# carlostojal/NDT-Net

Hardware: AMD Instinct MI355X
Metric: clouds/sec NDT preprocess+PointNet fwd, 100k pts->1000 NDs, batch=16 (higher is better)
Workload: dtype f64 NDT; PointNet fp32-accurate split-bf16x3 (6 products) on 11 per-point layers, fp32 MFMA on the K=16 first layers and the TNet / seg-bias FC layers

## Files before the change

include/ndnet_pointnet.h:

```cpp
#ifndef NDNET_POINTNET_H_
#define NDNET_POINTNET_H_
#include <stdint.h>

#ifdef __cplusplus
extern "C" {
#endif

#define NDNET_PN_MAX_LAYERS 5

typedef struct ndnet_pn_layer {
  const float* w;
  int64_t w_cloud_stride;
  const float* bias;
  int64_t bias_cloud_stride;
  int32_t K, N;
  int32_t relu;
  int32_t prec;
  int32_t fuse_next;
} ndnet_pn_layer;

typedef struct ndnet_pn_chain {
  const float* x;
  int32_t x_ld;
  int32_t in_cols;
  int32_t num_points;
  int32_t num_layers;
  ndnet_pn_layer L[NDNET_PN_MAX_LAYERS];
  int32_t mode;
  int32_t out_cols;
  float* gmax;
  int32_t gmax_ld;
  int32_t max_width;
  int32_t max_width2;
  float* out;
  float* clear;
  int64_t clear_count;
  const float* head_h2;
  int32_t head_ld, head_K;
  const float* head_w3;
  const float* head_b3;
  const float* head_basis;
  int32_t head_kin, head_nout;
  float* head_t1;
  const float* fold_t2;
  int32_t fold_ld;
  float* fold_out_w;
  float* fold_out_b;
} ndnet_pn_chain;

int ndnet_pn_chain_run(const ndnet_pn_chain *args, int batch, void *stream);
int ndnet_pn_chain_run_t32(const ndnet_pn_chain *args, int batch, void *stream);

int ndnet_pn_debug_stamps(unsigned long long *host, int wgs);
int ndnet_pn_debug_stamps_clear(void);

int ndnet_pn_fc_run(const float *in, int ld_in, const float *W, const float *bias, float *out, int ld_out,
                    int batch, int K, int N, int relu, void *stream);
int ndnet_pn_fc_mfma_run(const float *in, int ld_in, const float *Wf, const float *bias, float *out, int ld_out,
                         int batch, int K, int N, int relu, void *stream);
int ndnet_pn_cls_head_run(const float *in, int ld_in, const float *Wf, const float *bias, float *probs,
                          int ld_probs, float *logits, int ld_logits, int batch, int K, int N, int out_cols,
                          float *clear, int64_t clear_count, void *stream);
#define NDNET_FOLD_WT 0
#define NDNET_FOLD_FRAG 1
#define NDNET_FOLD_FRAG6 2
#define NDNET_FOLD_ROWS 3
#define NDNET_FOLD_BASIS 4
#define NDNET_FOLD_BIAS 5
typedef struct ndnet_pn_fold_job {
  const float *w;
  const float *bias;
  const float *gamma, *beta, *mean, *var;
  void *out;
  int32_t kind;
  int32_t N, K;
  int32_t ld, k0;
  int32_t Kp, Np;
  int32_t eye;
  float eps;
  int32_t reserved;
  int64_t block0;
} ndnet_pn_fold_job;
int ndnet_pn_fold_prepare(ndnet_pn_fold_job *host_jobs, int num_jobs, int64_t *num_blocks);
int ndnet_pn_fold_run(const ndnet_pn_fold_job *device_jobs, int num_jobs, int64_t num_blocks, void *stream);

int ndnet_pn_head3_run(const float *h2, int ld_h, const float *W3, const float *b3, const float *basis,
                       float *t1, float *w1f, int batch, int K, int kin, int nout, void *stream);

int ndnet_pn_fold_t2_run(const float *w1f, int w1_stride, const float *b1, const float *t2, int t2_ld, float *outf,
                         float *outb, int batch, void *stream);

#ifdef __cplusplus
}
#endif

#endif
```

ndt-net_amd/csrc/pointnet_kernels.hip:

```cpp
#include <hip/hip_runtime.h>
#include <math.h>
#include <stdint.h>
#include <stdio.h>
#include <stdlib.h>

#include "../../include/ndnet_pointnet.h"

namespace {

#ifndef NDNET_PN_TILE
#define NDNET_PN_TILE 64
#endif
constexpr int kP = NDNET_PN_TILE;
#ifndef NDNET_PN_WAVES
#define NDNET_PN_WAVES (NDNET_PN_TILE / 4)
#endif
constexpr int kWaves = NDNET_PN_WAVES;
constexpr int kThreads = 64 * kWaves;
constexpr int kRowBlocks = kP / 16;
static_assert(kP == 64 || kP == 32, "64- or 32-point tiles");
constexpr int kFuseNC = 64;
constexpr int kPadF = 8;
constexpr int kPadB = 16;
#ifndef NDNET_PN_PLANE_SWZ
// ... 1155 lines not shown
  return ((int64_t)((n >> 4) * KG + (k >> 4)) * 64 + ((k >> 2) & 3) * 16 + (n & 15)) * 4 + (k & 3);
}

template <int WPO>
__global__ void __launch_bounds__(256) k_pn_fc_split(const float* __restrict__ in, int ld_in,
                                                     const float* __restrict__ W, const float* __restrict__ bias,
                                                     float* __restrict__ out, int ld_out, int B, int N, int relu) {
  constexpr int K = 256 * WPO, OPW = 4 / WPO;
  __shared__ float s_part[4][16];
  const int lane = threadIdx.x & 63, wave = threadIdx.x >> 6;
  const int o = wave / WPO, wq = wave % WPO;
  const int n = blockIdx.x * OPW + o;
  const int nn = n < N ? n : N - 1;
  const int c4 = wq * 64 + lane;
  const f32x4 wv = reinterpret_cast<const f32x4*>(W + (int64_t)nn * K)[c4];
  f32x4 xv[16];
#pragma unroll
  for (int b = 0; b < 16; b++) xv[b] = reinterpret_cast<const f32x4*>(in + (int64_t)(b < B ? b : 0) * ld_in)[c4];
  float acc[16];
#pragma unroll
  for (int b = 0; b < 16; b++) {
    const f32x4 pr = xv[b] * wv;
    acc[b] = (pr[0] + pr[1]) + (pr[2] + pr[3]);
  }
#pragma unroll
  for (int b = 0; b < 16; b++)
    for (int off = 32; off > 0; off >>= 1) acc[b] += __shfl_xor(acc[b], off, 64);
  if (WPO > 1) {
    if (lane < 16) {
      float v = 0.0f;
#pragma unroll
      for (int b = 0; b < 16; b++) v = lane == b ? acc[b] : v;
      s_part[wave][lane] = v;
    }
    __syncthreads();
    if (wq != 0) return;
    if (lane < 16) {
      float v = 0.0f;
#pragma unroll
      for (int q = 0; q < WPO; q++) v += s_part[wave + q][lane];
      acc[0] = v;
    }
  } else if (lane < 16) {
    float v = 0.0f;
#pragma unroll
    for (int b = 0; b < 16; b++) v = lane == b ? acc[b] : v;
    acc[0] = v;
  }
  if (lane < B && n < N) {
    float v = acc[0] + bias[n];
    if (relu) v = fmaxf(v, 0.0f);
    out[(int64_t)lane * ld_out + n] = v;
  }
}

__global__ void __launch_bounds__(1024) k_pn_fold_t2(const float* __restrict__ w1f, int w1_stride,
                                                     const float* __restrict__ b1, const float* __restrict__ t2,
                                                     int t2_ld, float* __restrict__ outf, float* __restrict__ outb) {
  const int b = blockIdx.x, e = threadIdx.x;
  __shared__ float s_w[13 * 64];
  __shared__ float s_t[64 * 64];
  {
    const float* wb = w1f + (int64_t)b * w1_stride;
    if (e < 16 * 64) {
      const int cb = e >> 8, ln = (e >> 2) & 63, k = 4 * (ln >> 4) + (e & 3), n = 16 * cb + (ln & 15);
      const float v = wb[e];
      if (k < 12) s_w[k * 64 + n] = v;
    }
    if (e < 64) s_w[12 * 64 + e] = b1[e];
    const f32x4* tb = reinterpret_cast<const f32x4*>(t2 + (int64_t)b * t2_ld);
    reinterpret_cast<f32x4*>(s_t)[e] = tb[e];
  }
  __syncthreads();
  if (e < 13 * 64) {
    const int r = e >> 6, n = e & 63;
    float acc = 0.0f;
#pragma unroll 16
    for (int i = 0; i < 64; i++) acc = fmaf(s_w[r * 64 + i], s_t[i * 64 + n], acc);
    if (r < 12) outf[(int64_t)b * 1024 + ((((n >> 4) * 64 + ((r >> 2) & 3) * 16 + (n & 15)) << 2) + (r & 3))] = acc;
    else outb[(int64_t)b * 64 + n] = acc;
  }
}

__global__ void __launch_bounds__(256) k_pn_head3(const float* __restrict__ h2, int ld_h, const float* __restrict__ W3,
                                                  const float* __restrict__ b3, const float* __restrict__ basis,
                                                  float* __restrict__ t1_out, float* __restrict__ w1f, int K, int kin,
                                                  int nout) {
  __shared__ float s_t[9];
  const int b = blockIdx.x;
  const int lane = threadIdx.x & 63, wave = threadIdx.x >> 6;
  const float* h = h2 + (int64_t)b * ld_h;
  for (int o = wave; o < 9; o += 4) {
    float acc = 0.0f;
    for (int k = lane; k < K; k += 64) acc += h[k] * W3[(int64_t)o * K + k];
    for (int off = 32; off > 0; off >>= 1) acc += __shfl_xor(acc, off, 64);
    if (lane == 0) {
      s_t[o] = acc + b3[o];
      t1_out[b * 9 + o] = acc + b3[o];
    }
  }
  const int M = kin * nout, total = 16 * nout;
  auto kn = [&](int e, int& k, int& n) {
    const int cb = e >> 8, ln = (e >> 2) & 63;
    k = 4 * (ln >> 4) + (e & 3);
    n = 16 * cb + (ln & 15);
  };
  constexpr int kE = 4;
  float bas[kE][9];
#pragma unroll
  for (int i = 0; i < kE; i++) {
    const int e = threadIdx.x + i * blockDim.x;
    int k, n;
    kn(e, k, n);
#pragma unroll
    for (int a = 0; a < 9; a++) bas[i][a] = (e < total && k < kin) ? basis[a * M + k * nout + n] : 0.0f;
  }
  __syncthreads();
#pragma unroll
  for (int i = 0; i < kE; i++) {
    const int e = threadIdx.x + i * blockDim.x;
    if (e < total) {
      float acc = 0.0f;
#pragma unroll
      for (int a = 0; a < 9; a++) acc += s_t[a] * bas[i][a];
      w1f[(int64_t)b * total + e] = acc;
    }
  }
  for (int e = threadIdx.x + kE * blockDim.x; e < total; e += blockDim.x) {
    int k, n;
    kn(e, k, n);
    float acc = 0.0f;
    if (k < kin) {
#pragma unroll
      for (int a = 0; a < 9; a++) acc += s_t[a] * basis[a * M + k * nout + n];
    }
    w1f[(int64_t)b * total + e] = acc;
  }
}

#if NDNET_PN_TILE == 64
constexpr int kFoldThreads = 256;

__device__ inline uint16_t fold_bf16(float x) {
  uint32_t u = __float_as_uint(x);
  if ((u & 0x7fffffffu) > 0x7f800000u) return (uint16_t)((u >> 16) | 0x40u);
  return (uint16_t)((u + 0x7fffu + ((u >> 16) & 1u)) >> 16);
}

__device__ inline float fold_w(const ndnet_pn_fold_job& J, int n, int k) {
#pragma clang fp contract(off)
  if (n >= J.N || k >= J.K) return 0.0f;
  const float w = J.w[(int64_t)n * J.ld + J.k0 + k];
  if (!J.gamma) return w;
  return w * (J.gamma[n] / sqrtf(J.var[n] + J.eps));
}

__host__ __device__ inline int64_t fold_units(const ndnet_pn_fold_job& J) {
  switch (J.kind) {
    case NDNET_FOLD_WT: return (int64_t)J.Kp * J.Np;
    case NDNET_FOLD_FRAG: return (int64_t)J.Kp * J.Np / 4;
    case NDNET_FOLD_FRAG6: return (int64_t)J.Kp * J.Np / 8;
    case NDNET_FOLD_ROWS: return (int64_t)J.N * J.K;
    case NDNET_FOLD_BASIS: return (int64_t)9 * J.K * J.N;
    default: return J.Np;
  }
}
// ... 75 lines not shown
    }
  }
}
#endif

#if NDNET_PN_TILE == 64
int fc_mfma_cbw(int nb, int ngmax) {
  static const int cap = [] {
    const char* e = getenv("NDNET_PN_FC_CBW");
    return e ? atoi(e) : 4;
  }();
  for (int c = cap >= 4 ? 4 : cap >= 2 ? 2 : 1; c > 1; c >>= 1)
    if (nb % c == 0 && nb / c >= 32 && ngmax * c <= kFcMaxG) return c;
  return 1;
}
#endif

}

extern "C" {

#if NDNET_PN_TILE == 64
int ndnet_pn_fc_mfma_run(const float* in, int ld_in, const float* Wf, const float* bias, float* out, int ld_out,
                         int batch, int K, int N, int relu, void* stream) {
  if (!in || !Wf || !bias || !out || batch <= 0 || batch > 16 || K <= 0 || K % 16 || K > 16 * kFcWaves * kFcMaxG ||
      N <= 0 || N % 16 || ld_in % 4 || ld_in < K || ld_out < N || ((uintptr_t)in | (uintptr_t)Wf) % 16)
    return -20;
  const int KG = K / 16, nb = N / 16, ngmax = (KG + kFcWaves - 1) / kFcWaves;
  const int cbw = fc_mfma_cbw(nb, ngmax);
  const f32x4* wf = reinterpret_cast<const f32x4*>(Wf);
  hipStream_t st = (hipStream_t)stream;
  if (cbw == 4)
    k_pn_fc_mfma<4><<<nb / 4, kFcWaves * 64, 0, st>>>(in, ld_in, wf, bias, out, ld_out, batch, KG, relu);
  else if (cbw == 2)
    k_pn_fc_mfma<2><<<nb / 2, kFcWaves * 64, 0, st>>>(in, ld_in, wf, bias, out, ld_out, batch, KG, relu);
  else
    k_pn_fc_mfma<1><<<nb, kFcWaves * 64, 0, st>>>(in, ld_in, wf, bias, out, ld_out, batch, KG, relu);
  return hipGetLastError() == hipSuccess ? 0 : -21;
}

int ndnet_pn_cls_head_run(const float* in, int ld_in, const float* Wf, const float* bias, float* probs, int ld_probs,
                          float* logits, int ld_logits, int batch, int K, int N, int out_cols, float* clear,
                          int64_t clear_count, void* stream) {
  if (!in || !Wf || !bias || !probs || batch <= 0 || K <= 0 || K % 16 || K > 16 * kClsMaxG || N <= 0 || N % 16 ||
      N > 1024 || out_cols < 1 || out_cols > N || ld_in % 4 || ld_in < K || ld_probs < out_cols ||
      (logits && ld_logits < out_cols) || ((uintptr_t)in | (uintptr_t)Wf) % 16 || clear_count < 0 ||
      (!clear && clear_count))
    return -20;
  k_pn_cls_head<<<(batch + 15) / 16, kClsWaves * 64, (size_t)16 * N * sizeof(float), (hipStream_t)stream>>>(
      in, ld_in, reinterpret_cast<const f32x4*>(Wf), bias, probs, ld_probs, logits, ld_logits, batch, K / 16, N,
      out_cols, clear, clear_count);
  return hipGetLastError() == hipSuccess ? 0 : -21;
}

int ndnet_pn_fc_run(const float* in, int ld_in, const float* W, const float* bias, float* out, int ld_out, int batch,
                    int K, int N, int relu, void* stream) {
  if (!in || !W || !bias || !out || batch <= 0 || batch > 16 || K <= 0 || K % 4 || N <= 0 || ld_in % 4 ||
      ld_in < K || ld_out < N || ((uintptr_t)in | (uintptr_t)W) % 16)
    return -20;
  hipStream_t st = (hipStream_t)stream;
  switch (K % 256 == 0 && K <= 1024 ? K / 256 : 0) {
    case 2: k_pn_fc_split<2><<<(N + 1) / 2, 256, 0, st>>>(in, ld_in, W, bias, out, ld_out, batch, N, relu); break;
    case 4: k_pn_fc_split<4><<<N, 256, 0, st>>>(in, ld_in, W, bias, out, ld_out, batch, N, relu); break;
    default: k_pn_fc<<<(N + 3) / 4, 256, 0, st>>>(in, ld_in, W, bias, out, ld_out, batch, K, N, relu);
  }
  return hipGetLastError() == hipSuccess ? 0 : -21;
}

int ndnet_pn_head3_run(const float* h2, int ld_h, const float* W3, const float* b3, const float* basis, float* t1,
                       float* w1f, int batch, int K, int kin, int nout, void* stream) {
  if (!h2 || !W3 || !b3 || !basis || !t1 || !w1f || batch <= 0 || K <= 0 || ld_h < K || kin <= 0 || kin > 16 ||
      nout <= 0 || nout % 16)
    return -20;
  k_pn_head3<<<batch, 256, 0, (hipStream_t)stream>>>(h2, ld_h, W3, b3, basis, t1, w1f, K, kin, nout);
  return hipGetLastError() == hipSuccess ? 0 : -21;
}

int ndnet_pn_fold_t2_run(const float* w1f, int w1_stride, const float* b1, const float* t2, int t2_ld, float* outf,
                         float* outb, int batch, void* stream) {
  if (!w1f || !b1 || !t2 || !outf || !outb || batch <= 0 || w1_stride < 1024 || t2_ld < 4096 || t2_ld % 4 ||
      (uintptr_t)t2 % 16)
    return -20;
  k_pn_fold_t2<<<batch, 1024, 0, (hipStream_t)stream>>>(w1f, w1_stride, b1, t2, t2_ld, outf, outb);
  return hipGetLastError() == hipSuccess ? 0 : -21;
}

int ndnet_pn_fold_prepare(ndnet_pn_fold_job* jobs, int num_jobs, int64_t* num_blocks) {
  if (!jobs || num_jobs <= 0 || !num_blocks) return -20;
  int64_t blocks = 0;
  for (int i = 0; i < num_jobs; i++) {
    ndnet_pn_fold_job& J = jobs[i];
    const bool bn = J.gamma != nullptr;
    if (!J.out || (uintptr_t)J.out % 16 || J.kind < NDNET_FOLD_WT || J.kind > NDNET_FOLD_BIAS || J.N <= 0 ||
        (bn && (!J.beta || !J.mean || !J.var || !(J.eps >= 0.0f))) || (!bn && (J.beta || J.mean || J.var)))
      return -20;
    if (J.kind == NDNET_FOLD_BIAS) {
      if (!J.bias || J.Np < J.N || J.eye < 0 || (J.eye > 0 && J.eye * J.eye != J.N)) return -20;
    } else {
      if (!J.w || J.K <= 0 || J.k0 < 0 || J.ld < J.k0 + J.K) return -20;
      if (J.kind == NDNET_FOLD_WT && (J.Kp < J.K || J.Np < J.N)) return -20;
      if (J.kind == NDNET_FOLD_FRAG && (J.Kp < J.K || J.Np < J.N || J.Kp % 16 || J.Np % 16)) return -20;
      if (J.kind == NDNET_FOLD_FRAG6 && (J.Kp < J.K || J.Np < J.N || J.Kp % 32 || J.Np % 16)) return -20;
      if (J.kind == NDNET_FOLD_BASIS && J.K != 12) return -20;
    }
    J.block0 = blocks;
    blocks += (fold_units(J) + kFoldThreads - 1) / kFoldThreads;
  }
  if (blocks <= 0 || blocks > 0x7fffffff) return -20;
  *num_blocks = blocks;
  return 0;
}

int ndnet_pn_fold_run(const ndnet_pn_fold_job* jobs, int num_jobs, int64_t num_blocks, void* stream) {
  if (!jobs || num_jobs <= 0 || num_blocks <= 0 || num_blocks > 0x7fffffff) return -20;
  k_pn_fold<<<(unsigned)num_blocks, kFoldThreads, 0, (hipStream_t)stream>>>(jobs, num_jobs);
  return hipGetLastError() == hipSuccess ? 0 : -21;
}


int ndnet_pn_debug_stamps_clear(void) {
#ifdef NDNET_PN_STAMPS
  static unsigned long long zeros[kStampWgs][16];
  return hipMemcpyToSymbol(HIP_SYMBOL(g_pn_stamps), zeros, sizeof(zeros)) == hipSuccess ? 0 : -21;
#else
  return -20;
#endif
}

int ndnet_pn_debug_stamps(unsigned long long* host, int wgs) {
#ifdef NDNET_PN_STAMPS
  if (!host || wgs <= 0 || wgs > kStampWgs) return -20;
  if (hipDeviceSynchronize() != hipSuccess) return -21;
  return hipMemcpyFromSymbol(host, HIP_SYMBOL(g_pn_stamps), (size_t)wgs * 16 * sizeof(unsigned long long)) ==
                 hipSuccess ? 0 : -21;
#else
  (void)host; (void)wgs;
  return -20;
#endif
}
#endif

#define PN_ARG_FAIL()                                                                          \
  do {                                                                                         \
    fprintf(stderr, "ndnet_amd: chain launch: invalid argument (pointnet_kernels.hip:%d)\n", __LINE__); \
    return -20;                                                                                \
  } while (0)

#if NDNET_PN_TILE == 64
int ndnet_pn_chain_run(const ndnet_pn_chain* args, int batch, void* stream) {
#else
int ndnet_pn_chain_run_t32(const ndnet_pn_chain* args, int batch, void* stream) {
#endif
  if (!args || batch <= 0 || args->num_layers < 1 || args->num_layers > NDNET_PN_MAX_LAYERS || args->num_points <= 0 ||
      args->in_cols < 1 || args->in_cols > args->L[0].K || args->in_cols > args->x_ld)
    PN_ARG_FAIL();
  int w[2] = {args->L[0].K, 0};
  int pw1 = 0;
  bool has_fuse = false;
  int planes = 0, qprec = 0;
  int smode = 0;
  for (int l = 0; l < args->num_layers; l++) {
    const ndnet_pn_layer& L = args->L[l];
    if (!L.w || !L.bias || L.K <= 0 || L.K % 16 || L.N <= 0 || L.N % 32 || (L.N > 32 && L.N % 64) ||
        ((uintptr_t)L.w % 16) ||
        L.w_cloud_stride % 4)
      PN_ARG_FAIL();
// ... 88 lines not shown
```

ndt-net_amd/ndnet/_lib.py:

```python
from __future__ import annotations

import ctypes
import os

import torch

PKG = os.path.dirname(os.path.abspath(__file__))
ROOT = os.path.dirname(PKG)
LIB_PATH = os.environ.get("NDNET_AMD_LIB") or os.path.join(ROOT, "lib", "libndnet_amd.so")

NDNET_OK = 0
NDNET_ERR_ARG = -20
NDNET_ERR_HIP = -21
NDNET_ERR_SYNC = -22
POINT_FILL = {"none": 0, "nearest": 1}
SEG_CONF_LDS_MAX_COLS = 63
FPS_THREADS = 512
FPS_LDS_POINTS = {"float32": 12288, "float64": 6144}
FPS_REG_POINTS = {"float32": 100352, "float64": 49152}


class NdtStats(ctypes.Structure):
    _fields_ = [
        ("rc", ctypes.c_int32),
# ... 54 lines not shown
    "free_nds": (None, [_P, _UL]),
    "free_kl_divergences": (None, [_P]),
    "print_matrix": (None, [_P, _I, _I]),
    "ndnet_ndt_plan_create": (_I, [_I, _U64, _U64, _I, _U64, ctypes.POINTER(_P)]),
    "ndnet_ndt_plan_destroy": (None, [_P]),
    "ndnet_ndt_set_path": (_I, [_P, _I]),
    "ndnet_ndt_get_path": (_I, [_P]),
    "ndnet_ndt_get_front_lanes": (_I, [_P, ctypes.POINTER(_I), ctypes.POINTER(_I)]),
    "ndnet_ndt_take_sync_failures": (_I, [_P]),
    "ndnet_ndt_set_cu_share": (_I, [_P, _I, _I]),
    "ndnet_ndt_set_exact_counts": (_I, [_P, _I]),
    "ndnet_ndt_set_front_staged": (_I, [_P, _I]),
    "ndnet_ndt_get_front_staged": (_I, [_P]),
    "ndnet_ndt_set_run_part": (_I, [_P, _I]),
    "ndnet_ndt_set_lazy_list": (_I, [_P, _I]),
    "ndnet_ndt_set_heavy_threshold": (_I, [_P, ctypes.c_uint32]),
    "ndnet_ndt_set_welford_form": (_I, [_P, _I]),
    "ndnet_ndt_get_welford_form": (_I, [_P]),
    "ndnet_ndt_debug_set_sync_timeout": (_I, [_P, ctypes.c_uint64]),
    "ndnet_ndt_run": (_I, [_P, _P, _P, _P, _P, _P, _P]),
    "ndnet_ndt_run_f64": (_I, [_P, _P, _P, _P, _P, _P, _P, _P, _P]),
    "ndnet_ndt_prune": (_I, [_P, _P, _U64, _P, _P, _P, _P, _P, _P]),
    "ndnet_ndt_point_rows": (_I, [_P, _P, _P, _P, _U64, _I, _P]),
    "ndnet_ndt_run_counts": (_I, [_P, _P, _P, _P, _P, _P, _P, _P]),
    "ndnet_ndt_run_f64_counts": (_I, [_P, _P, _P, _P, _P, _P, _P, _P, _P, _P]),
    "ndnet_ndt_point_rows_counts": (_I, [_P, _P, _P, _P, _U64, _I, _P, _P]),
    "ndnet_seg_point_labels": (_I, [_P, _P, _I, _U64, _U64, _I, ctypes.c_int32, _P, _P, _P]),
    "ndnet_seg_point_labels_u8": (_I, [_P, _P, _I, _U64, _U64, _I, ctypes.c_uint8, _P, _P, _P]),
    "ndnet_seg_confusion": (_I, [_P, _P, _U64, _I, _P, _P]),
    "ndnet_seg_row_hist": (_I, [_P, _P, _I, _U64, _U64, _I, ctypes.c_int32, _P, _P]),
    "ndnet_fps_run": (_I, [_P, _I, _U64, _U64, _P, _P, _P, _P, _P]),
    "ndnet_fps_run_f64": (_I, [_P, _I, _U64, _U64, _P, _P, _P, _P, _P]),
    "ndnet_nearest_sample_run": (_I, [_P, _I, _U64, _P, _P, _U64, _P, _P, _P, _P]),
    "ndnet_pn_transform3_run": (_I, [_P, ctypes.c_int64, _P, _P, ctypes.c_int64, _I, _U64, _P]),
    "ndnet_aug_work_bytes": (ctypes.c_size_t, [_I, _U64]),
    "ndnet_aug_run": (_I, [_P, _P, _P, _P, _I, _U64, _P, _P, _P, _P, _P, _P, _P]),
    "ndnet_pts_unpack_i16": (_I, [_P, _P, _I, _U64, _P, _P, _P]),
    "ndnet_ndt_debug_dump": (_I, [_P, _I, _P, _P, _P, _P, _P, _P, _P, _P, _P, _P, _P, _P]),
    "ndnet_ndt_debug_set_epoch": (_I, [_P, ctypes.c_uint32]),
    "ndnet_ndt_debug_set_kl_fuse": (_I, [_P, _I]),
    "ndnet_ndt_debug_set_list_sort": (_I, [_P, _I]),
    "ndnet_ndt_debug_get_list_sort": (_I, [_P]),
    "ndnet_ndt_debug_kl_marks": (_I, [_P, _P]),
    "ndnet_ndt_debug_front_marks": (_I, [_P, _P]),
    "ndnet_ndt_debug_wq_marks": (_I, [_P, _P, ctypes.POINTER(ctypes.c_uint32)]),
    "ndnet_debug_lu_chain": (_I, [_P, ctypes.c_uint32, _I, _P, _P, _P, _P]),
    "ndnet_ndt_debug_front_wg_marks": (_I, [_P, _P, ctypes.POINTER(_I)]),
    "ndnet_ndt_set_timing": (_I, [_P, _I]),
    "ndnet_ndt_stage_ms": (_I, [_P, _P]),
    "ndnet_amd_version": (ctypes.c_char_p, []),
}


def lib() -> ctypes.CDLL:
    global _lib
    if _lib is None:
        if not os.path.exists(LIB_PATH):
            raise RuntimeError(f"{LIB_PATH} is missing: build it with `make -C {ROOT}` "
                               "(there is no CPU fallback)")
        _lib = ctypes.CDLL(LIB_PATH)
        for name, (res, args) in EXPORTS.items():
            fn = getattr(_lib, name)
            fn.restype = res
            fn.argtypes = args
        for name, (res, args) in {**POINTNET_EXPORTS, **TRAIN_EXPORTS}.items():
            fn = getattr(_lib, name)
            fn.restype = res
            fn.argtypes = args
    return _lib


POINTNET_EXPORTS: dict = {
    "ndnet_pn_chain_run": (_I, [_P, _I, _P]),
    "ndnet_pn_chain_run_t32": (_I, [_P, _I, _P]),
    "ndnet_pn_debug_stamps": (_I, [_P, _I]),
    "ndnet_pn_debug_stamps_clear": (_I, []),
    "ndnet_ply_count": (_I, [ctypes.c_char_p, _I, ctypes.POINTER(_U64)]),
    "ndnet_ply_read": (_I, [ctypes.c_char_p, _I, _I, _P, _P, _U64, ctypes.POINTER(_U64), _I]),
    "ndnet_pn_fc_run": (_I, [_P, _I, _P, _P, _P, _I, _I, _I, _I, _I, _P]),
    "ndnet_pn_fc_mfma_run": (_I, [_P, _I, _P, _P, _P, _I, _I, _I, _I, _I, _P]),
    "ndnet_pn_cls_head_run": (_I, [_P, _I, _P, _P, _P, _I, _P, _I, _I, _I, _I, _I, _P, ctypes.c_int64, _P]),
    "ndnet_pn_head3_run": (_I, [_P, _I, _P, _P, _P, _P, _P, _I, _I, _I, _I, _P]),
    "ndnet_pn_fold_t2_run": (_I, [_P, _I, _P, _P, _I, _P, _P, _I, _P]),
    "ndnet_pn_fold_prepare": (_I, [_P, _I, ctypes.POINTER(ctypes.c_int64)]),
    "ndnet_pn_fold_run": (_I, [_P, _I, ctypes.c_int64, _P]),
}


_I64 = ctypes.c_int64

TRAIN_EXPORTS: dict = {
    "ndnet_tr_gemm": (_I, [_P, _P, _P, _P, _I64, _I, _I, _I, _I64, _I64, _I64, _I64, _I64, _I64, _I, _I, _I, _I, _I,
                           _I, _P]),
    "ndnet_tr_sum_parts": (_I, [_P, _P, _I64, _I, _P]),
    "ndnet_tr_sum_parts_2d": (_I, [_P, _P, _I64, _I64, _I64, _I, _P]),
    "ndnet_tr_bn_fwd": (_I, [_P, _P, _P, _P, _P, _P, _P, _P, _I, _I, _I, ctypes.c_float, ctypes.c_float, _I, _P, _P,
                             _P, _P]),
    "ndnet_tr_bn_bwd": (_I, [_P, _P, _P, _P, _P, _P, _P, _P, _P, _P, _I, _I, _I, _I, _P, _P]),
    "ndnet_tr_chan_sum": (_I, [_P, _P, _I, _I, _I, _P]),
    "ndnet_tr_row_sum": (_I, [_P, _P, _I64, _I, _P]),
    "ndnet_tr_argmax_match": (_I, [_P, _P, _I64, _I, _P, _P]),
    "ndnet_tr_argmax_match_cm": (_I, [_P, _P, _I, _I, _I, _P, _P, _P]),
    "ndnet_row_argmax": (_I, [_P, _I64, _I, _P, _P]),
    "ndnet_tr_fc_fwd": (_I, [_P, _P, _P, _P, _P, _P, _P, _P, _P, _P, _P, _I, _I, _I, _I64, ctypes.c_float,
                             ctypes.c_float, _I, _I, _P, _P]),
    "ndnet_tr_fc_bwd_w": (_I, [_P, _P, _P, _P, _P, _P, _P, _P, _P, _P, _P, _P, _I, _I, _I, _I64, _I, _P]),
    "ndnet_tr_fc_bwd_x": (_I, [_P, _P, _P, _P, _I, _I, _I, _I64, _I, _P]),
    "ndnet_tr_point_transform": (_I, [_P, _P, _I, _P, _I, _P, _I, _I, _P]),
    "ndnet_tr_point_transform_bwd": (_I, [_P, _P, _I, _P, _I, _P, _I, _I, _P]),
    "ndnet_tr_log_softmax_c": (_I, [_P, _P, _I, _I, _I, _P]),
    "ndnet_tr_log_softmax_c_bwd": (_I, [_P, _P, _P, _I, _I, _I, _P]),
    "ndnet_tr_nll_onehot": (_I, [_P, _P, _P, _P, _I, _I, _I, _P]),
    "ndnet_tr_nll_onehot_bwd": (_I, [_P, _P, _P, _I, _I, _I, _P]),
    "ndnet_tr_nll_hist": (_I, [_P, _P, _P, _P, _P, _I, _I, _I, _P]),
    "ndnet_tr_nll_hist_bwd": (_I, [_P, _P, _P, _P, _I, _I, _I, _P]),
    "ndnet_tr_hist_match_cm": (_I, [_P, _P, _I, _I, _I, _P, _P, _P]),
    "ndnet_tr_adam": (_I, [_I, _P, _P, _P, _P, _P, _P, _P, ctypes.c_double, ctypes.c_double, ctypes.c_double,
                           ctypes.c_double, _P]),
}


def require_gpu() -> None:
    if not torch.cuda.is_available():
        raise RuntimeError("ndnet_amd needs a ROCm GPU (gfx950); none is visible and there is no CPU fallback")


def check(rc: int, what: str) -> None:
    if rc != NDNET_OK:
        raise RuntimeError(f"{what} failed with code {rc}")


def stream_ptr(device: torch.device | None = None) -> int:
    return torch.cuda.current_stream(device).cuda_stream
```

ndt-net_amd/ndnet/models/pointnet_hip.py:

```python
from __future__ import annotations

import ctypes
import os

import torch

from .. import _lib

MAX_LAYERS = 5
CHAIN_NAMES = ("A: TNet(3) 3-64-128-1024 + max", "B: conv1(t1) + TNet(64) 64-64-128-1024 + max",
               "C: conv1, conv2(t2), conv3 + max", "D: seg head 64-512-256-128-(C+1) + log_softmax")

chain_timing = None

MODES = {"x6": 1, "fp32": 1, "x3": 2, "bf16": 3}
PRECISION = SPLIT_BF16 = X6_PREC = None


def set_precision(mode: str) -> None:
    global PRECISION, SPLIT_BF16, X6_PREC
    if mode not in MODES:
        raise ValueError(f"unknown PointNet precision mode {mode!r}")
    PRECISION = mode
    SPLIT_BF16 = mode != "fp32"
# ... 298 lines not shown
                and all(t.is_contiguous() and t.dtype == torch.float32 for t in tensors if t.is_floating_point()))

    def refold(self) -> None:
        dev = self.c1wT.device
        if self._dev_jobs is None:
            arr = (_FoldJob * len(self.jobs))()
            for J, (kind, out, layer, bn, k0, K, Kp, Np, eye) in zip(arr, self.jobs):
                J.kind, J.out, J.N, J.K, J.ld, J.k0 = kind, out.data_ptr(), layer.weight.shape[0], K, \
                    layer.weight.shape[1], k0
                J.Kp, J.Np, J.eye = Kp, Np, eye
                if kind == 5:
                    J.bias = layer.bias.data_ptr()
                else:
                    J.w = layer.weight.data_ptr()
                if bn is not None:
                    J.gamma, J.beta = bn.weight.data_ptr(), bn.bias.data_ptr()
                    J.mean, J.var, J.eps = bn.running_mean.data_ptr(), bn.running_var.data_ptr(), bn.eps
            blocks = ctypes.c_int64()
            _lib.check(_lib.lib().ndnet_pn_fold_prepare(arr, len(arr), ctypes.byref(blocks)), "ndnet_pn_fold_prepare")
            self._dev_jobs = torch.frombuffer(bytearray(bytes(arr)), dtype=torch.uint8).to(dev)
            self._blocks = blocks.value
        rc = _lib.lib().ndnet_pn_fold_run(self._dev_jobs.data_ptr(), len(self.jobs), self._blocks,
                                          _lib.stream_ptr(dev))
        _lib.check(rc, "ndnet_pn_fold_run")


def _tensors(m) -> list:
    return list(m.parameters()) + list(m.buffers())


def _signature(tensors) -> tuple:
    return tuple((t.data_ptr(), t._version) for t in tensors)


def _fc_head(g: torch.Tensor, t: dict, dim: int, h1: torch.Tensor, h2: torch.Tensor, out: torch.Tensor):
    torch.addmm(t["c1"], g, t["f1"].t(), out=h1).relu_()
    torch.addmm(t["c2"], h1, t["f2"].t(), out=h2).relu_()
    torch.addmm(t["c3"], h2, t["f3"].t(), out=out)
    return out.view(-1, dim, dim)


def _build_chain(n: int, in_cols: int, layers, relus, mode: int, gmax=None, out_cols=0, fuse=(),
                 x_ld: int = 12) -> "_Chain":
    ch = _Chain()
    ch.x_ld = x_ld
    ch.in_cols = in_cols
    ch.num_points = n
    ch.num_layers = len(layers)
    widths = [layers[0][3], 8]
    for i, (w, stride, b, K, N, *prec) in enumerate(layers):
        L = ch.L[i]
        L.prec = prec[0] if prec else 0
        L.w = w.data_ptr()
        L.w_cloud_stride = stride
        L.K, L.N = K, N
        L.bias = b.data_ptr()
        L.bias_cloud_stride = b.stride(0) if b.dim() == 2 else 0
        L.relu = relus[i]
        L.fuse_next = 1 if i in fuse else 0
        if i in fuse:
            continue
        if i + 1 < len(layers) or mode == 1:
            widths[(i + 1) & 1] = max(widths[(i + 1) & 1], N)
    ch.mode = mode
    ch.out_cols = out_cols
    ch.gmax = gmax.data_ptr() if gmax is not None else None
    ch.gmax_ld = gmax.stride(0) if gmax is not None else 0
    ch.max_width, ch.max_width2 = widths
    return ch


TILE32 = os.environ.get("NDNET_PN_TILE32", "1") == "1"
_cus = {}


def _use_t32(B: int, n: int, device) -> bool:
    if not TILE32:
        return False
    if device not in _cus:
        _cus[device] = torch.cuda.get_device_properties(device).multi_processor_count
    return 2 * B * ((n + 63) // 64) <= _cus[device]


def _run_chain(ch: "_Chain", x: torch.Tensor, out=None) -> None:
    assert x.stride(1) == ch.x_ld and x.stride(2) == 1 and x.dtype == torch.float32
    ch.x = x.data_ptr()
    ch.out = out.data_ptr() if out is not None else None
    if _use_t32(x.shape[0], x.shape[1], x.device):
        rc = _lib.lib().ndnet_pn_chain_run_t32(ctypes.byref(ch), x.shape[0], _lib.stream_ptr(x.device))
        _lib.check(rc, "ndnet_pn_chain_run_t32")
        return
    rc = _lib.lib().ndnet_pn_chain_run(ctypes.byref(ch), x.shape[0], _lib.stream_ptr(x.device))
    _lib.check(rc, "ndnet_pn_chain_run")


def _chain_torch(x: torch.Tensor, n: int, in_cols: int, layers, relus, mode: int, gmax=None, out=None,
                 out_cols=0, fuse=()) -> None:
    h = x[..., :in_cols].float()
    k0 = layers[0][0].shape[-2]
    h = torch.nn.functional.pad(h, (0, k0 - in_cols))
    for i, (w, b) in enumerate(layers):
        h = torch.matmul(h, w[..., : h.shape[-1], :]) + (b[:, None, :] if b.dim() == 2 else b)
        if relus[i]:
            h = torch.relu(h)
    if mode == 0:
        gmax.copy_(torch.maximum(gmax, h.amax(dim=1)))
    else:
        out.copy_(torch.log_softmax(h[..., :out_cols], dim=2))


class _Workspace:

    def __init__(self, W: _Folded, B: int, N: int, dev, mode: str = None) -> None:
        self.W = W
        self.mode = PRECISION if mode is None else mode
        f32 = dict(dtype=torch.float32, device=dev)
        Fp = W.C_tail[0].shape[1]
        self.gbuf = torch.full((B, 2048 + Fp), float("-inf"), **f32)
        self.g1, self.g2, self.g3 = self.gbuf[:, :1024], self.gbuf[:, 1024:2048], self.gbuf[:, 2048:]
        self.h1, self.h2 = torch.empty((B, 512), **f32), torch.empty((B, 256), **f32)
        self.t1, self.t2 = torch.empty((B, 9), **f32), torch.empty((B, 4096), **f32)
        self.cvec = torch.empty((B, 512), **f32)
        kin = 3 if W.baseline else 12
        self.w1T = None if W.baseline else torch.empty((B, 12, 64), **f32)
        self.w1t2 = torch.empty((B, kin, 64), **f32)
        self.b1t2 = torch.empty((B, 64), **f32)
        self.w1f = None if W.baseline else torch.empty((B, 16 * 64), **f32)
        self.w1t2f = torch.zeros((B, 16 * 64), **f32)
        if W.baseline:
            self.xt = torch.zeros((B, N, 4), **f32)
            self.pts = None
        first = (W.c1T16, W.c1b) if W.baseline else (self.w1T, W.c1b)
        self.specs = [
            (3, W.A, (1, 1, 1), 0, dict(gmax=self.g1)),
            (kin, [first] + W.B_tail, (0, 1, 1, 1), 0, dict(gmax=self.g2)),
            (kin, [(self.w1t2, self.b1t2), W.C_mid, W.C_tail], (0, 0, 0), 0, dict(gmax=self.g3)),
        ]
        if W.seg:
            self.specs.append((kin, [(self.w1t2, self.b1t2), (W.s1aT, self.cvec)] + W.D_tail, (0, 1, 1, 1, 0), 1,
                               dict(out_cols=W.C1, fuse=(1,))))
        self.N = N
        self.structs = {}

    def hip_layers(self, mode: str) -> list:
        W = self.W

        def shared(wb):
            w, b = wb
            if mode != "fp32" and id(w) in W.frag6:
                return (W.frag6[id(w)], 0, b, w.shape[0], w.shape[1], MODES[mode])
            return (W.frag[id(w)], 0, b, w.shape[0], w.shape[1])

        L1 = shared((W.c1T16, W.c1b)) if W.baseline else (self.w1f, self.w1f.stride(0), W.c1b, 16, 64)
        LC = (self.w1t2f, self.w1t2f.stride(0), self.b1t2, 16, 64) if FOLD_T2_KERNEL and not W.baseline else L1
        layers = [
            [shared(x) for x in W.A],
            [L1] + [shared(x) for x in W.B_tail],
            [LC, shared(W.C_mid), shared(W.C_tail)],
        ]
        if W.seg:
            layers.append([(self.w1t2f, self.w1t2f.stride(0), self.b1t2, 16, 64), shared((W.s1aT, self.cvec))] +
                          [shared(x) for x in W.D_tail])
        return layers

    def chain(self, i: int, x: torch.Tensor, chain_fn=None, out=None) -> None:
        in_cols, layers, relus, mode, kw = self.specs[i]
        if chain_fn is not None:
            kw = dict(kw)
            if out is not None:
                kw["out"] = out
            chain_fn(x, self.N, in_cols, layers, relus, mode, **kw)
            return
        structs = self.structs.get(self.mode)
        W = self.W
        if structs is None:
            x_lds = (3, 4, 4, 4) if W.baseline else (12, 12, 12, 12)
            structs = self.structs[self.mode] = [_build_chain(self.N, s[0], hl, s[2], s[3], x_ld=xl, **s[4])
                                                 for s, hl, xl in zip(self.specs, self.hip_layers(self.mode), x_lds)]
            if W.seg:
                structs[3].clear = self.gbuf.data_ptr()
                structs[3].clear_count = self.gbuf.numel()
            if HEAD3_IN_CHAIN and not W.baseline:
                cb = structs[1]
                cb.head_h2, cb.head_ld, cb.head_K = self.h2.data_ptr(), self.h2.stride(0), self.h2.shape[1]
                cb.head_w3, cb.head_b3 = W.t1["f3"].data_ptr(), W.t1["c3"].data_ptr()
                cb.head_basis, cb.head_kin, cb.head_nout = W.t1_basis.data_ptr(), 12, 64
                cb.head_t1 = self.t1.data_ptr()
            if not FOLD_T2_KERNEL or W.baseline:
                cc = structs[2]
                cc.fold_t2, cc.fold_ld = self.t2.data_ptr(), self.t2.stride(0)
                cc.fold_out_w, cc.fold_out_b = self.w1t2f.data_ptr(), self.b1t2.data_ptr()
        if chain_timing is not None:
            e0, e1 = torch.cuda.Event(enable_timing=True), torch.cuda.Event(enable_timing=True)
            e0.record()
            _run_chain(structs[i], x, out)
            e1.record()
            chain_timing.append((i, e0, e1))
        else:
            _run_chain(structs[i], x, out)


def _folded(model):
    cache = model._hip
    if cache is None:
        tensors = _tensors(model)
        cache = model._hip = {"tensors": tensors, "sig": None, "stale": False}
    sig = _signature(cache["tensors"])
    cur = _tensors(model)
    replaced = len(cur) != len(cache["tensors"]) or any(a is not b for a, b in zip(cur, cache["tensors"]))
    if replaced or cache["sig"] != sig or cache["stale"]:
        W = cache.get("W")
        if W is not None and W.can_refold(_tensors(model)):
            W.refold()
        else:
            cache.update(tensors=_tensors(model), W=_Folded(model), ws={})
            sig = _signature(cache["tensors"])
        cache.update(sig=sig, stale=False)
    return cache


FOLD_T2_KERNEL = os.environ.get("NDNET_PN_FOLD_T2", "kernel") == "kernel"
HEAD3_IN_CHAIN = os.environ.get("NDNET_PN_HEAD3", "chain") == "chain"

FC_MFMA = os.environ.get("NDNET_PN_FC", "mfma") == "mfma"


def _fc(x: torch.Tensor, w: torch.Tensor, b: torch.Tensor, out: torch.Tensor, relu: bool, wf=None) -> None:
    B = x.shape[0]
    st = _lib.stream_ptr(x.device)
    for c0 in range(0, B, 16):
        n = min(16, B - c0)
        if FC_MFMA and wf is not None:
            rc = _lib.lib().ndnet_pn_fc_mfma_run(x[c0].data_ptr(), x.stride(0), wf.data_ptr(), b.data_ptr(),
                                                 out[c0].data_ptr(), out.stride(0), n, _pad(w.shape[1], 16),
                                                 w.shape[0], 1 if relu else 0, st)
            _lib.check(rc, "ndnet_pn_fc_mfma_run")
        else:
            rc = _lib.lib().ndnet_pn_fc_run(x[c0].data_ptr(), x.stride(0), w.data_ptr(), b.data_ptr(),
                                            out[c0].data_ptr(), out.stride(0), n, w.shape[1], w.shape[0],
                                            1 if relu else 0, st)
            _lib.check(rc, "ndnet_pn_fc_run")


def _glue_hip(W, ws, B: int):
    st = lambda: _lib.stream_ptr(ws.gbuf.device)

    def fc(x, w, b, out, relu):
        _fc(x, w, b, out, relu, W.fcf.get(id(w)))

    def head_a():
        t = W.t1
        fc(ws.g1, t["f1"], t["c1"], ws.h1, True)
        fc(ws.h1, t["f2"], t["c2"], ws.h2, True)
        if HEAD3_IN_CHAIN:
            return
        for c0 in range(0, B, 16):
            n = min(16, B - c0)
            rc = _lib.lib().ndnet_pn_head3_run(ws.h2[c0].data_ptr(), ws.h2.stride(0), t["f3"].data_ptr(),
                                               t["c3"].data_ptr(), W.t1_basis.data_ptr(), ws.t1[c0].data_ptr(),
                                               ws.w1f[c0].data_ptr(), n, 256, 12, 64, st())
            _lib.check(rc, "ndnet_pn_head3_run")

    def head_a_points():
        t = W.t1
        fc(ws.g1, t["f1"], t["c1"], ws.h1, True)
        fc(ws.h1, t["f2"], t["c2"], ws.h2, True)
        _fc(ws.h2, t["f3"], t["c3"], ws.t1, False, None)
        rc = _lib.lib().ndnet_pn_transform3_run(ws.pts.data_ptr(), ws.pts.stride(1), ws.t1.data_ptr(),
                                                ws.xt.data_ptr(), ws.xt.stride(1), B, ws.pts.shape[1], st())
        _lib.check(rc, "ndnet_pn_transform3_run")

    def head_b():
        t = W.t2
        fc(ws.g2, t["f1"], t["c1"], ws.h1, True)
        fc(ws.h1, t["f2"], t["c2"], ws.h2, True)
        fc(ws.h2, t["f3"], t["c3"], ws.t2, False)
        if FOLD_T2_KERNEL and not W.baseline:
            rc = _lib.lib().ndnet_pn_fold_t2_run(ws.w1f.data_ptr(), ws.w1f.stride(0), W.c1b.data_ptr(),
                                                 ws.t2.data_ptr(), ws.t2.stride(0), ws.w1t2f.data_ptr(),
                                                 ws.b1t2.data_ptr(), B, st())
            _lib.check(rc, "ndnet_pn_fold_t2_run")

    def seg_bias():
        fc(ws.g3[:, : W.F], W.s1g, W.s1b, ws.cvec, False)

    def cls_head(out):
        fc(ws.g3[:, : W.F], W.h1w, W.h1b, ws.h1, True)
        fc(ws.h1, W.h2w, W.h2b, ws.h2, True)
        rc = _lib.lib().ndnet_pn_cls_head_run(ws.h2.data_ptr(), ws.h2.stride(0), W.h3f.data_ptr(), W.h3b.data_ptr(),
                                              out.data_ptr(), out.stride(0), None, 0, B, ws.h2.shape[1], W.Cp, W.C,
                                              ws.gbuf.data_ptr(), ws.gbuf.numel(), st())
        _lib.check(rc, "ndnet_pn_cls_head_run")

    return (head_a_points if W.baseline else head_a), head_b, (seg_bias if W.seg else cls_head)


def _glue_torch(W, ws, B: int):
    def head_a():
        t1 = _fc_head(ws.g1, W.t1, 3, ws.h1, ws.h2, ws.t1)
        torch.matmul(t1.reshape(B, 9), W.t1_basis, out=ws.w1T.view(B, 12 * 64))

    def head_a_points():
        t1 = _fc_head(ws.g1, W.t1, 3, ws.h1, ws.h2, ws.t1)
        ws.xt[..., :3] = torch.nan_to_num(torch.bmm(ws.pts, t1.transpose(1, 2)), nan=0.0)
# ... 85 lines not shown
```

Measured before the change: 88750.

## Collapse third backbone chain into folded affine pool12 kernel with max-pool

Adds a kernel that folds the chain-2 layers (first layer with t2 fold, mid 64x128, tail 128xF, apparently linear with no ReLU between) into one 12->F affine map per cloud, computed in f64 MFMA. It then runs a single K=12 fp32 MFMA per point tile with a running max to produce the global max-pool. This drops the per-point 64- and 128-wide layers of chain 2, removing most of that stage's FLOPs and intermediate traffic. It is enabled by default in x6/fp32 mode. The main risk is numerical: the composed weights are rounded to fp32 and the K=12 product is a single fp32 MFMA rather than split-bf16x3.

```diff
diff --git a/include/ndnet_pointnet.h b/include/ndnet_pointnet.h
--- a/include/ndnet_pointnet.h
+++ b/include/ndnet_pointnet.h
@@ -90,6 +90,11 @@
 int ndnet_pn_fold_t2_run(const float *w1f, int w1_stride, const float *b1, const float *t2, int t2_ld, float *outf,
                          float *outb, int batch, void *stream);
 
+int ndnet_pn_pool12_run(const float *x, int x_ld, int num_points, const float *w0f, int64_t w0_stride,
+                        const float *b0, int64_t b0_stride, const float *w_mid, const float *b_mid,
+                        const float *w_tail, const float *b_tail, int F, int Fp, float *gmax, int gmax_ld,
+                        int batch, void *stream);
+
 #ifdef __cplusplus
 }
 #endif
diff --git a/ndt-net_amd/csrc/pointnet_kernels.hip b/ndt-net_amd/csrc/pointnet_kernels.hip
--- a/ndt-net_amd/csrc/pointnet_kernels.hip
+++ b/ndt-net_amd/csrc/pointnet_kernels.hip
@@ -1261,6 +1261,158 @@
   }
 }
 
+#if NDNET_PN_TILE == 64
+typedef double f64x4 __attribute__((ext_vector_type(4)));
+constexpr int kP12Waves = 16;
+constexpr int kP12Pre = 4;
+constexpr int kP12Pitch = 130;
+
+__device__ inline void p12_rows(const float* __restrict__ xb, int x_ld, int n, int tile, int kq, int cl, float (&v)[3]) {
+  const int p = min(16 * tile + cl, n - 1);
+  const float* r = xb + (int64_t)p * x_ld + kq;
+#pragma unroll
+  for (int s = 0; s < 3; s++) v[s] = r[4 * s];
+}
+
+__device__ inline void p12_clean(int n, int tile, int cl, float (&v)[3]) {
+  const bool in = 16 * tile + cl < n;
+#pragma unroll
+  for (int s = 0; s < 3; s++) v[s] = (in & (fabsf(v[s]) < INFINITY)) ? v[s] : NAN;
+}
+
+__global__ void __launch_bounds__(kP12Waves * 64) k_pn_pool12(
+    const float* __restrict__ x, int x_ld, int n, const float* __restrict__ w0f, int64_t w0_stride,
+    const float* __restrict__ b0, int64_t b0_stride, const float* __restrict__ w_mid,
+    const float* __restrict__ b_mid, const float* __restrict__ w_tail, const float* __restrict__ b_tail, int Fp,
+    float* __restrict__ gmax, int gmax_ld) {
+  __shared__ double s_m[13 * kP12Pitch];
+  __shared__ float s_wc[13 * 64];
+  __shared__ float s_red[kP12Waves * 64];
+  const int b = blockIdx.y, c0 = 64 * blockIdx.x;
+  const int lane = threadIdx.x & 63, kq = lane >> 4, cl = lane & 15;
+  const int wave = __builtin_amdgcn_readfirstlane((int)threadIdx.x >> 6);
+  const int tiles = (n + 15) >> 4;
+  const float* xb = x + (int64_t)b * n * x_ld;
+
+  float xp[kP12Pre][3];
+#pragma unroll
+  for (int i = 0; i < kP12Pre; i++) p12_rows(xb, x_ld, n, wave + kP12Waves * i, kq, cl, xp[i]);
+  float tw[32];
+
+  if (wave < 8) {
+    const float* wb = w0f + (int64_t)b * w0_stride;
+    const float* bb = b0 + (int64_t)b * b0_stride;
+    float a[16], bw[16];
+#pragma unroll
+    for (int ks = 0; ks < 16; ks++) {
+      const int i = 4 * ks + kq;
+      const float* src = cl < 12 ? wb + ((((i >> 4) * 64 + ((cl >> 2) & 3) * 16 + (i & 15)) << 2) + (cl & 3)) : bb + i;
+      a[ks] = *src;
+      bw[ks] = w_mid[i * 128 + 16 * wave + cl];
+    }
+#pragma unroll
+    for (int ks = 0; ks < 16; ks++) a[ks] = cl < 13 ? a[ks] : 0.0f;
+    f64x4 acc0 = {0.0, 0.0, 0.0, 0.0}, acc1 = {0.0, 0.0, 0.0, 0.0};
+#pragma unroll
+    for (int ks = 0; ks < 16; ks += 2) {
+      acc0 = __builtin_amdgcn_mfma_f64_16x16x4f64((double)a[ks], (double)bw[ks], acc0, 0, 0, 0);
+      acc1 = __builtin_amdgcn_mfma_f64_16x16x4f64((double)a[ks + 1], (double)bw[ks + 1], acc1, 0, 0, 0);
+    }
+#pragma unroll
+    for (int q = 0; q < 4; q++) {
+      const int row = kq + 4 * q, col = 16 * wave + cl;
+      double v = acc0[q] + acc1[q];
+      if (row == 12) v += (double)b_mid[col];
+      if (row < 13) s_m[row * kP12Pitch + col] = v;
+    }
+  } else if (wave < 12) {
+    const int tc = min(c0 + 16 * (wave - 8) + cl, Fp - 1);
+#pragma unroll
+    for (int ks = 0; ks < 32; ks++) tw[ks] = w_tail[(int64_t)(4 * ks + kq) * Fp + tc];
+  }
+  __syncthreads();
+  if (wave >= 8 && wave < 12) {
+    f64x4 acc0 = {0.0, 0.0, 0.0, 0.0}, acc1 = {0.0, 0.0, 0.0, 0.0};
+#pragma unroll
+    for (int ks = 0; ks < 32; ks += 2) {
+      const double a0 = s_m[min(cl, 12) * kP12Pitch + 4 * ks + kq], a1 = s_m[min(cl, 12) * kP12Pitch + 4 * ks + 4 + kq];
+      acc0 = __builtin_amdgcn_mfma_f64_16x16x4f64(cl < 13 ? a0 : 0.0, (double)tw[ks], acc0, 0, 0, 0);
+      acc1 = __builtin_amdgcn_mfma_f64_16x16x4f64(cl < 13 ? a1 : 0.0, (double)tw[ks + 1], acc1, 0, 0, 0);
+    }
+#pragma unroll
+    for (int q = 0; q < 4; q++) {
+      const int row = kq + 4 * q, col = 16 * (wave - 8) + cl;
+      double v = acc0[q] + acc1[q];
+      if (row == 12) v += (double)b_tail[min(c0 + col, Fp - 1)];
+      if (row < 13) s_wc[row * 64 + col] = (float)v;
+    }
+  }
+  __syncthreads();
+
+  float wc[4][3];
+#pragma unroll
+  for (int cb = 0; cb < 4; cb++)
+#pragma unroll
+    for (int s = 0; s < 3; s++) wc[cb][s] = s_wc[(4 * s + kq) * 64 + 16 * cb + cl];
+  float m[4][4];
+#pragma unroll
+  for (int cb = 0; cb < 4; cb++)
+#pragma unroll
+    for (int r = 0; r < 4; r++) m[cb][r] = -INFINITY;
+  auto tile = [&](int t, float (&xv)[3]) {
+    p12_clean(n, t, cl, xv);
+    f32x4 acc[4];
+#pragma unroll
+    for (int cb = 0; cb < 4; cb++) acc[cb] = f32x4{0.f, 0.f, 0.f, 0.f};
+#pragma unroll
+    for (int s = 0; s < 3; s++)
+#pragma unroll
+      for (int cb = 0; cb < 4; cb++) acc[cb] = __builtin_amdgcn_mfma_f32_16x16x4f32(wc[cb][s], xv[s], acc[cb], 0, 0, 0);
+#pragma unroll
+    for (int cb = 0; cb < 4; cb++)
+#pragma unroll
+      for (int r = 0; r < 4; r++) m[cb][r] = fmaxf(m[cb][r], acc[cb][r]);
+  };
+#pragma unroll
+  for (int i = 0; i < kP12Pre; i++)
+    if (wave + kP12Waves * i < tiles) tile(wave + kP12Waves * i, xp[i]);
+  for (int t = wave + kP12Waves * kP12Pre; t < tiles; t += kP12Waves) {
+    float xv[3];
+    p12_rows(xb, x_ld, n, t, kq, cl, xv);
+    tile(t, xv);
+  }
+  float* mv = &m[0][0];
+#pragma unroll
+  for (int i = 0; i < 8; i++) {
+    const bool hi = cl & 8;
+    mv[i] = fmaxf(hi ? mv[i + 8] : mv[i], xor_row<8>(hi ? mv[i] : mv[i + 8]));
+  }
+#pragma unroll
+  for (int i = 0; i < 4; i++) {
+    const bool hi = cl & 4;
+    mv[i] = fmaxf(hi ? mv[i + 4] : mv[i], xor_row<4>(hi ? mv[i] : mv[i + 4]));
+  }
+#pragma unroll
+  for (int i = 0; i < 2; i++) {
+    const bool hi = cl & 2;
+    mv[i] = fmaxf(hi ? mv[i + 2] : mv[i], xor_row<2>(hi ? mv[i] : mv[i + 2]));
+  }
+  {
+    const bool hi = cl & 1;
+    mv[0] = fmaxf(hi ? mv[1] : mv[0], xor_row<1>(hi ? mv[0] : mv[1]));
+  }
+  s_red[wave * 64 + 16 * (cl >> 2) + 4 * kq + (cl & 3)] = mv[0];
+  __syncthreads();
+  if (threadIdx.x < 64) {
+    const int c = threadIdx.x;
+    float mm = s_red[c];
+#pragma unroll
+    for (int w = 1; w < kP12Waves; w++) mm = fmaxf(mm, s_red[w * 64 + c]);
+    if (c0 + c < Fp) gmax[(int64_t)b * gmax_ld + c0 + c] = mm > -INFINITY ? (mm + s_wc[12 * 64 + c]) + 0.0f : -INFINITY;
+  }
+}
+#endif
+
 __global__ void __launch_bounds__(256) k_pn_head3(const float* __restrict__ h2, int ld_h, const float* __restrict__ W3,
                                                   const float* __restrict__ b3, const float* __restrict__ basis,
                                                   float* __restrict__ t1_out, float* __restrict__ w1f, int K, int kin,
@@ -1502,6 +1654,18 @@
       (uintptr_t)t2 % 16)
     return -20;
   k_pn_fold_t2<<<batch, 1024, 0, (hipStream_t)stream>>>(w1f, w1_stride, b1, t2, t2_ld, outf, outb);
+  return hipGetLastError() == hipSuccess ? 0 : -21;
+}
+
+int ndnet_pn_pool12_run(const float* x, int x_ld, int num_points, const float* w0f, int64_t w0_stride, const float* b0,
+                        int64_t b0_stride, const float* w_mid, const float* b_mid, const float* w_tail,
+                        const float* b_tail, int F, int Fp, float* gmax, int gmax_ld, int batch, void* stream) {
+  if (!x || !w0f || !b0 || !w_mid || !b_mid || !w_tail || !b_tail || !gmax || batch <= 0 || batch > 65535 ||
+      num_points <= 0 || x_ld < 12 || x_ld % 4 || w0_stride < 1024 || b0_stride < 64 || F <= 0 || F > Fp ||
+      (Fp != 32 && Fp % 64) || gmax_ld < Fp)
+    return -20;
+  k_pn_pool12<<<dim3((Fp + 63) / 64, batch), kP12Waves * 64, 0, (hipStream_t)stream>>>(
+      x, x_ld, num_points, w0f, w0_stride, b0, b0_stride, w_mid, b_mid, w_tail, b_tail, Fp, gmax, gmax_ld);
   return hipGetLastError() == hipSuccess ? 0 : -21;
 }
 
diff --git a/ndt-net_amd/ndnet/_lib.py b/ndt-net_amd/ndnet/_lib.py
--- a/ndt-net_amd/ndnet/_lib.py
+++ b/ndt-net_amd/ndnet/_lib.py
@@ -160,6 +160,8 @@
     "ndnet_pn_cls_head_run": (_I, [_P, _I, _P, _P, _P, _I, _P, _I, _I, _I, _I, _I, _P, ctypes.c_int64, _P]),
     "ndnet_pn_head3_run": (_I, [_P, _I, _P, _P, _P, _P, _P, _I, _I, _I, _I, _P]),
     "ndnet_pn_fold_t2_run": (_I, [_P, _I, _P, _P, _I, _P, _P, _I, _P]),
+    "ndnet_pn_pool12_run": (_I, [_P, _I, _I, _P, ctypes.c_int64, _P, ctypes.c_int64, _P, _P, _P, _P, _I, _I, _P, _I,
+                                 _I, _P]),
     "ndnet_pn_fold_prepare": (_I, [_P, _I, ctypes.POINTER(ctypes.c_int64)]),
     "ndnet_pn_fold_run": (_I, [_P, _I, ctypes.c_int64, _P]),
 }
diff --git a/ndt-net_amd/ndnet/models/pointnet_hip.py b/ndt-net_amd/ndnet/models/pointnet_hip.py
--- a/ndt-net_amd/ndnet/models/pointnet_hip.py
+++ b/ndt-net_amd/ndnet/models/pointnet_hip.py
@@ -404,7 +404,30 @@
     return 2 * B * ((n + 63) // 64) <= _cus[device]
 
 
-def _run_chain(ch: "_Chain", x: torch.Tensor, out=None) -> None:
+class _Pool12:
+
+    def __init__(self, ws: "_Workspace") -> None:
+        W = ws.W
+        (w_mid, b_mid), (w_tail, b_tail) = W.C_mid, W.C_tail
+        assert w_mid.shape == (64, 128) and w_mid.is_contiguous() and w_tail.shape[0] == 128 and w_tail.is_contiguous()
+        self.tensors = (ws.w1t2f, ws.b1t2, w_mid, b_mid, w_tail, b_tail, ws.g3)
+        self.n, self.F, self.Fp = ws.N, W.F, w_tail.shape[1]
+        self.args = (ws.w1t2f.data_ptr(), ws.w1t2f.stride(0), ws.b1t2.data_ptr(), ws.b1t2.stride(0),
+                     w_mid.data_ptr(), b_mid.data_ptr(), w_tail.data_ptr(), b_tail.data_ptr(), self.F, self.Fp,
+                     ws.g3.data_ptr(), ws.g3.stride(0))
+
+
+def _run_pool12(blk: "_Pool12", x: torch.Tensor) -> None:
+    B, n, _ = x.shape
+    assert n == blk.n and x.stride(2) == 1 and x.stride(0) == n * x.stride(1) and x.dtype == torch.float32
+    rc = _lib.lib().ndnet_pn_pool12_run(x.data_ptr(), x.stride(1), n, *blk.args, B, _lib.stream_ptr(x.device))
+    _lib.check(rc, "ndnet_pn_pool12_run")
+
+
+def _run_chain(ch, x: torch.Tensor, out=None) -> None:
+    if isinstance(ch, _Pool12):
+        _run_pool12(ch, x)
+        return
     assert x.stride(1) == ch.x_ld and x.stride(2) == 1 and x.dtype == torch.float32
     ch.x = x.data_ptr()
     ch.out = out.data_ptr() if out is not None else None
@@ -463,6 +486,10 @@
                                dict(out_cols=W.C1, fuse=(1,))))
         self.N = N
         self.structs = {}
+        self.pool12 = None
+
+    def uses_pool12(self) -> bool:
+        return BACKBONE == "pool12" and FOLD_T2_KERNEL and not self.W.baseline and self.mode in ("x6", "fp32")
 
     def hip_layers(self, mode: str) -> list:
         W = self.W
@@ -512,14 +539,19 @@
                 cc = structs[2]
                 cc.fold_t2, cc.fold_ld = self.t2.data_ptr(), self.t2.stride(0)
                 cc.fold_out_w, cc.fold_out_b = self.w1t2f.data_ptr(), self.b1t2.data_ptr()
+        blk = structs[i]
+        if i == 2 and self.uses_pool12():
+            if self.pool12 is None:
+                self.pool12 = _Pool12(self)
+            blk = self.pool12
         if chain_timing is not None:
             e0, e1 = torch.cuda.Event(enable_timing=True), torch.cuda.Event(enable_timing=True)
             e0.record()
-            _run_chain(structs[i], x, out)
+            _run_chain(blk, x, out)
             e1.record()
             chain_timing.append((i, e0, e1))
         else:
-            _run_chain(structs[i], x, out)
+            _run_chain(blk, x, out)
 
 
 def _folded(model):
@@ -542,6 +574,9 @@
 
 
 FOLD_T2_KERNEL = os.environ.get("NDNET_PN_FOLD_T2", "kernel") == "kernel"
+BACKBONE = os.environ.get("NDNET_PN_BACKBONE", "pool12")
+if BACKBONE not in ("pool12", "chain"):
+    raise ValueError(f"NDNET_PN_BACKBONE must be 'pool12' or 'chain', not {BACKBONE!r}")
 HEAD3_IN_CHAIN = os.environ.get("NDNET_PN_HEAD3", "chain") == "chain"
 
 FC_MFMA = os.environ.get("NDNET_PN_FC", "mfma") == "mfma"
```

Measured after the change: 90050 (median of 6 runs). +1.5%, better.
